# sparisi/pvr_habitat

Measured on AMD Instinct MI355X. Metric: frames/sec embedded (ResNet50, 256x256), higher is better.
Workload: dtype f16; 1 GPU; configs[1]: ResNet50 (MoCo-v2 layout) frozen, 256x256 uint8 frames resident in HBM, batch 256/GPU, random-init synthetic weights, f16 storage / MFMA inputs with fp32 accumulation (the product default, inside the 1e-3 parity bound; configs[1] names bf16); global_batch=256, frame=256, chunk=256, batches_in_flight=2, parallelism=frame shards, no collective (dp1)

## Files before the change

include/pvr_hip.h:

```cpp
#ifndef PVR_HIP_H
#define PVR_HIP_H

#include <stddef.h>
#include <stdint.h>

#ifdef __cplusplus
extern "C" {
#endif

typedef int pvr_status;
#define PVR_OK 0
#define PVR_ERR_INVALID 1
#define PVR_ERR_MISSING_WEIGHT 2
#define PVR_ERR_HIP 3
#define PVR_ERR_STATE 4

#define PVR_BF16 0
#define PVR_F16 1
#define PVR_F32 2

#define PVR_ARCH_RESNET50 0
#define PVR_ARCH_RESNET50_L4 1
#define PVR_ARCH_RESNET50_L3 2
#define PVR_ARCH_CLIP_VIT_B32 3
// ... 72 lines not shown
                                        const void *w1f_dev, const float *b1f_dev, int32_t n, int32_t dtype, uint64_t *stamps_dev, void *hip_stream);
int64_t pvr_debug_bneck_frame_launches(void);
pvr_status pvr_debug_set_frame64(int32_t mode);
int64_t pvr_debug_bneck_frame64_launches(void);
pvr_status pvr_debug_bneck_frame64_stamps(const void *w1f_dev, const float *b1f_dev, const void *w2_dev, const float *b2_dev, const void *w3_dev, const float *b3_dev,
                                          const void *x_dev, void *y_dev, int32_t n, int32_t dtype, uint64_t *stamps_dev, void *hip_stream);
pvr_status pvr_op_conv_wfrag(const void *in_dev, const void *wgt_packed_dev, const float *bias_dev, const void *residual_dev, void *out_dev, int32_t n,
                             int32_t h, int32_t w, int32_t cin, int32_t cout, int32_t kh, int32_t kw, int32_t stride, int32_t pad, int32_t relu,
                             int32_t out_f32, int32_t dtype, void *hip_stream);
pvr_status pvr_op_conv2d_dual(const void *in_dev, const void *in2_dev, const void *wgt_dev, const float *bias_dev, void *out_dev, int32_t n, int32_t h,
                              int32_t w, int32_t cin, int32_t cout, int32_t kh, int32_t kw, int32_t stride, int32_t pad, int32_t h2, int32_t w2,
                              int32_t cin2, int32_t stride2, int32_t relu, int32_t dtype, void *hip_stream);
pvr_status pvr_op_conv_wfrag_pool(const void *in_dev, const void *wgt_packed_dev, const float *bias_dev, const void *residual_dev, float *pool_out_dev,
                                  int64_t pool_stride, int32_t n, int32_t cin, int32_t cout, int32_t dtype, void *hip_stream);
int64_t pvr_debug_conv_wfrag_launches(void);
pvr_status pvr_op_split16_pack_weights(const float *w_dev, void *out_dev, int32_t rows, int32_t k, void *hip_stream);
pvr_status pvr_op_conv2d_split16(const float *in_dev, const void *wgt_split_dev, const float *bias_dev, const float *residual_dev, float *out_dev, int32_t n,
                                 int32_t h, int32_t w, int32_t cin, int32_t cout, int32_t k, int32_t stride, int32_t pad, int32_t relu, void *hip_stream);
pvr_status pvr_op_conv2d_f32(const float *in_dev, const float *wgt_dev, const float *bias_dev, const float *residual_dev, float *out_dev, int32_t n,
                             int32_t h, int32_t w, int32_t cin, int32_t cout, int32_t k, int32_t stride, int32_t pad, int32_t relu, void *hip_stream);
int64_t pvr_debug_conv_split16_launches(void);
int64_t pvr_debug_chain_wave128_launches(void);
pvr_status pvr_debug_set_conv_algo(int32_t algo);
pvr_status pvr_file_sizes(const char *const *paths, int32_t n, int64_t *sizes, int32_t threads);
pvr_status pvr_read_files(const char *const *paths, int32_t n, uint8_t *dst, const int64_t *offsets, int32_t threads);
pvr_status pvr_stage_copy(void *dst, const void *src, int64_t rows, int64_t row_bytes, int64_t src_row_stride, int64_t run_bytes,
                          int64_t run_stride, int32_t threads);
int64_t pvr_png_scratch_bytes(int32_t n, int32_t h, int32_t w);
pvr_status pvr_png_decode(const uint8_t *files_dev, const int64_t *offsets_dev, int32_t n, int32_t h, int32_t w, uint8_t *out_dev,
                          uint8_t *scratch_dev, int64_t scratch_bytes, int32_t *status_dev, void *hip_stream);
// ... 15 lines not shown
```

pvr_habitat_amd/_lib.py:

```python
import ctypes as C
import os

_HERE = os.path.dirname(os.path.abspath(__file__))
LIB_PATH = os.environ.get('PVR_LIB') or os.path.join(_HERE, 'lib', 'libpvr_hip.so')

PVR_BF16, PVR_F16, PVR_F32 = 0, 1, 2
ARCH_RESNET50, ARCH_RESNET50_L4, ARCH_RESNET50_L3 = 0, 1, 2


class EncoderDesc(C.Structure):
    _fields_ = [('arch', C.c_int32), ('dtype', C.c_int32), ('max_batch', C.c_int32), ('chunk', C.c_int32),
                ('resize', C.c_int32), ('crop', C.c_int32), ('mean', C.c_float * 3), ('std_', C.c_float * 3)]


_lib = None

_SIGS = {
    'pvr_version': (C.c_char_p, []),
    'pvr_has_experiments': (C.c_int32, []),
    'pvr_debug_stem_u8_geometry_ok': (C.c_int32, [C.c_void_p, C.c_int32, C.c_int32, C.c_int32, C.c_int32]),
    'pvr_encoder_set_host_backend': (C.c_int, [C.c_void_p, C.c_int32]),
    'pvr_stage_copy': (C.c_int, [C.c_void_p, C.c_void_p, C.c_int64, C.c_int64, C.c_int64, C.c_int64, C.c_int64, C.c_int32]),
    'pvr_last_error': (C.c_size_t, [C.c_char_p, C.c_size_t]),
    'pvr_encoder_create': (C.c_int, [C.POINTER(EncoderDesc), C.POINTER(C.c_void_p)]),
# ... 21 lines not shown
    'pvr_encoder_profile_span': (C.c_int, [C.c_void_p, C.c_void_p, C.c_int32, C.c_int32, C.c_int32, C.c_void_p, C.c_int64, C.c_void_p, C.c_int32, C.c_int32,
                                           C.POINTER(C.c_float)]),
    'pvr_op_preprocess': (C.c_int, [C.c_void_p, C.c_int32, C.c_int32, C.c_int32, C.c_int32, C.c_int32, C.c_void_p, C.c_int32, C.c_void_p]),
    'pvr_op_stem': (C.c_int, [C.c_void_p, C.c_void_p, C.c_void_p, C.c_void_p, C.c_int32, C.c_int32, C.c_void_p]),
    'pvr_op_maxpool': (C.c_int, [C.c_void_p, C.c_void_p, C.c_int32, C.c_int32, C.c_int32, C.c_int32, C.c_int32, C.c_void_p]),
    'pvr_op_conv2d': (C.c_int, [C.c_void_p, C.c_void_p, C.c_void_p, C.c_void_p, C.c_void_p] + [C.c_int32] * 12 + [C.c_void_p]),
    'pvr_op_avgpool': (C.c_int, [C.c_void_p, C.c_void_p, C.c_int64, C.c_int32, C.c_int32, C.c_int32, C.c_int32, C.c_int32, C.c_void_p]),
    'pvr_debug_convert': (C.c_int, [C.c_void_p, C.c_void_p, C.c_int64, C.c_int32]),
    'pvr_op_bneck_frame': (C.c_int, [C.c_void_p] * 13 + [C.c_int32] * 3 + [C.c_void_p]),
    'pvr_debug_bneck_frame_launches': (C.c_int64, []),
    'pvr_debug_set_frame64': (C.c_int, [C.c_int32]),
    'pvr_debug_bneck_frame64_launches': (C.c_int64, []),
    'pvr_debug_bneck_frame64_stamps': (C.c_int, [C.c_void_p] * 8 + [C.c_int32] * 2 + [C.c_void_p] * 2),
    'pvr_op_conv_wfrag': (C.c_int, [C.c_void_p] * 5 + [C.c_int32] * 12 + [C.c_void_p]),
    'pvr_debug_conv_wfrag_launches': (C.c_int64, []),
    'pvr_op_conv_wfrag_pool': (C.c_int, [C.c_void_p] * 5 + [C.c_int64] + [C.c_int32] * 4 + [C.c_void_p]),
    'pvr_op_conv2d_dual': (C.c_int, [C.c_void_p] * 5 + [C.c_int32] * 15 + [C.c_void_p]),
    'pvr_op_pack_frag_weights': (C.c_int, [C.c_void_p, C.c_void_p, C.c_int32, C.c_int32, C.c_void_p]),
    'pvr_debug_bneck_frame_stamps': (C.c_int, [C.c_void_p] * 12 + [C.c_int32] * 2 + [C.c_void_p] * 2),
    'pvr_encoder_check_range': (C.c_int, [C.c_void_p, C.c_void_p, C.c_int32, C.c_int32, C.c_int32, C.c_void_p, C.c_int64, C.c_void_p, C.POINTER(C.c_int32)]),
    'pvr_encoder_debug_set_switch': (C.c_int, [C.c_void_p, C.c_char_p, C.c_int32]),
    'pvr_encoder_launch_kernel': (C.c_int32, [C.c_void_p, C.c_int32, C.c_int32, C.c_char_p, C.c_int32]),
    'pvr_op_split16_pack_weights': (C.c_int, [C.c_void_p, C.c_void_p, C.c_int32, C.c_int32, C.c_void_p]),
    'pvr_op_conv2d_split16': (C.c_int, [C.c_void_p] * 5 + [C.c_int32] * 9 + [C.c_void_p]),
    'pvr_op_conv2d_f32': (C.c_int, [C.c_void_p] * 5 + [C.c_int32] * 9 + [C.c_void_p]),
    'pvr_debug_conv_split16_launches': (C.c_int64, []),
    'pvr_debug_chain_wave128_launches': (C.c_int64, []),
    'pvr_op_nonfinite_flag': (C.c_int, [C.c_void_p, C.c_int64, C.c_int64, C.c_int64, C.c_void_p, C.c_void_p]),
}

# ... 38 lines not shown
```

pvr_habitat_amd/csrc/api.hip:

```cpp
#include <stdarg.h>
#include "encoder_internal.h"
#include "sample_rng.h"
#include <dlfcn.h>

namespace pvr {

static thread_local std::string g_err;

void set_error(const char *fmt, ...) {
    char buf[1024];
    va_list ap;
    va_start(ap, fmt);
    vsnprintf(buf, sizeof buf, fmt, ap);
    va_end(ap);
    g_err = buf;
}
const std::string &last_error() { return g_err; }

namespace {
typedef int (*roctx_push_fn)(const char *);
typedef int (*roctx_pop_fn)();
struct Roctx {
    roctx_push_fn push = nullptr;
    roctx_pop_fn pop = nullptr;
// ... 7 lines not shown
                if (push && pop) return;
                push = nullptr; pop = nullptr;
            }
        }
    }
};
const Roctx &roctx() { static Roctx r; return r; }
}
void trace_push(const char *name) { if (roctx().push) roctx().push(name); }
void trace_pop() { if (roctx().pop) roctx().pop(); }

long long conv_expand_launches();
long long bneck_frame_launches();
long long pp_persistent_launches();
long long conv_wfrag_launches();
long long conv_split16_launches();
long long chain_wave128_launches();
pvr_status launch_split16_pack(const float *w, void *out, int rows, int K, hipStream_t stream);
pvr_status launch_conv_split16(const float *in, const void *wsp, const float *bias, const float *res, float *out, int n, int h, int w, int cin,
                               int cout, int k, int stride, int pad, int relu, hipStream_t stream, float *out2 = nullptr, int n1 = 0, void *out16 = nullptr,
                               int terms = 3);

static void *g_zero = nullptr;
static pvr_status zero_page(void **out) {
    if (!g_zero) {
        PVR_HIP_TRY(hipMalloc(&g_zero, 256));
        PVR_HIP_TRY(hipMemset(g_zero, 0, 256));
        PVR_HIP_TRY(hipDeviceSynchronize());
    }
    *out = g_zero;
// ... 47 lines not shown
}
pvr_status pvr_op_conv2d_dual(const void *in, const void *in2, const void *wgt, const float *bias, void *out, int32_t n, int32_t h, int32_t w, int32_t cin,
                              int32_t cout, int32_t kh, int32_t kw, int32_t stride, int32_t pad, int32_t h2, int32_t w2, int32_t cin2, int32_t stride2,
                              int32_t relu, int32_t dtype, void *stream) {
    PVR_REQUIRE(in && in2 && wgt && bias && out && n > 0, "pvr_op_conv2d_dual: null argument");
    PVR_REQUIRE(dtype == PVR_BF16 || dtype == PVR_F16, "pvr_op_conv2d_dual: 16-bit storage types only");
    return launch_conv_pp256(op_switches(), in, wgt, bias, nullptr, out, n, h, w, cin, cout, kh, kw, stride, pad, relu, 0, 0, dtype, 224, (hipStream_t)stream, in2, h2, w2,
                             cin2, stride2);
}
pvr_status pvr_op_conv_wfrag_pool(const void *in, const void *wgt_packed, const float *bias, const void *residual, float *pool_out, int64_t pool_stride,
                                  int32_t n, int32_t cin, int32_t cout, int32_t dtype, void *stream) {
    PVR_REQUIRE(n > 0 && pool_out, "pvr_op_conv_wfrag_pool: empty input");
    return launch_conv_wfrag(op_switches(), in, wgt_packed, bias, residual, nullptr, n, 7, 7, cin, cout, 1, 1, 1, 0, 1, 1, dtype, (hipStream_t)stream, pool_out, pool_stride);
}
int64_t pvr_debug_conv_wfrag_launches(void) { return (int64_t)conv_wfrag_launches(); }
pvr_status pvr_op_split16_pack_weights(const float *w, void *out, int32_t rows, int32_t k, void *stream) {
    return launch_split16_pack(w, out, rows, k, (hipStream_t)stream);
}
pvr_status pvr_op_conv2d_split16(const float *in, const void *wgt_split, const float *bias, const float *residual, float *out, int32_t n, int32_t h,
                                 int32_t w, int32_t cin, int32_t cout, int32_t k, int32_t stride, int32_t pad, int32_t relu, void *stream) {
    PVR_REQUIRE(n > 0 && h > 0 && w > 0, "pvr_op_conv2d_split16: empty input");
    return launch_conv_split16(in, wgt_split, bias, residual, out, n, h, w, cin, cout, k, stride, pad, relu, (hipStream_t)stream);
}
pvr_status pvr_op_conv2d_f32(const float *in, const float *wgt, const float *bias, const float *residual, float *out, int32_t n, int32_t h, int32_t w,
                             int32_t cin, int32_t cout, int32_t k, int32_t stride, int32_t pad, int32_t relu, void *stream) {
    PVR_REQUIRE(in && wgt && bias && out && n > 0, "pvr_op_conv2d_f32: null argument");
    return launch_conv_f32(in, wgt, bias, residual, out, n, h, w, cin, cout, k, stride, pad, relu, (hipStream_t)stream);
}
int64_t pvr_debug_conv_split16_launches(void) { return (int64_t)conv_split16_launches(); }
int64_t pvr_debug_chain_wave128_launches(void) { return (int64_t)chain_wave128_launches(); }
// ... 98 lines not shown
```

pvr_habitat_amd/csrc/conv_wfrag.hip:

```cpp
#include "encoder_internal.h"

namespace pvr {

struct WFP {
    const u16 *in, *w, *res;
    const float *bias;
    void *out;
    int M, H, W, Cin, Cout, Ho, Wo, KH, KW, stride, pad, act;
    int MT, NCT;
    int nch, cpt;
    int KC;
    int ct_major;
    unsigned in_bytes, w_bytes, out_bytes, res_bytes;
    float *pool_out;
    long long pool_stride;
    int frames;
};

#define WF_LDS_PTR(off_) ((__attribute__((address_space(3))) void *)(smem + (off_)))

template <bool F16, int RES, bool OUT32, int KO = 0, bool POOL = false>
__global__ __launch_bounds__(512, 1) void conv_wfrag_kernel(WFP p) {
    typedef typename HT<F16>::V8 V8;
    constexpr int BMV = POOL ? 98 : 112;
    constexpr int BM = 112, NT = 7, XB = 16384;
    constexpr int OOB = 0x7ffffff0;
    extern __shared__ __attribute__((aligned(16))) char smem[];

    const int tid = threadIdx.x, lane = tid & 63;
    const int wave = __builtin_amdgcn_readfirstlane(tid >> 6);
    const int fr = lane & 15, fq = lane >> 4, sw = (fr >> 1) & 7;
    const int t = xcd_remap(blockIdx.x, gridDim.x);
    int mt, ct;
    if (p.ct_major) { ct = t / p.MT; mt = t - ct * p.MT; }
    else { mt = t / p.NCT; ct = t - mt * p.NCT; }
    const int m0 = mt * BMV, co0 = ct * 256;

    const auto rs_in = __builtin_amdgcn_make_buffer_rsrc(const_cast<u16 *>(p.in), 0, p.in_bytes, 0x00020000);
    const auto rs_w = __builtin_amdgcn_make_buffer_rsrc(const_cast<u16 *>(p.w), 0, p.w_bytes, 0x00020000);

    int a_off[2], a_m[2];
#pragma unroll
    for (int i = 0; i < 2; ++i) {
        const int g = wave + 8 * i, r = g * 8 + (lane >> 3);
        const int lch = (lane & 7) ^ ((r >> 1) & 7);
        const int m = m0 + r;
        const bool ok = g < BM / 8 && r < BMV && m < p.M;
        const int mm = ok ? m : 0;
        const int wo = mm % p.Wo, tq = mm / p.Wo, ho = tq % p.Ho, n = tq / p.Ho;
        const int hi0 = ho * p.stride - p.pad, wi0 = wo * p.stride - p.pad;
        a_off[i] = (((n * p.H + hi0) * p.W + wi0) * p.Cin + lch * 8) * 2;
// ... 71 lines not shown
    {                                                                                                          \
        asm volatile("s_waitcnt vmcnt(6)" ::: "memory");                                                        \
        if constexpr (!(KO & 4)) __builtin_amdgcn_s_barrier();                                                  \
        __builtin_amdgcn_sched_barrier(0);                                                                      \
        WF_LOAD_W1(WF_, 0, 0) WF_STEP(0, B_, BN_, W_)                                                           \
        WF_LOAD_W1(WF_, 0, 1) WF_STEP(1, B_, BN_, W_)                                                           \
        WF_LOAD_W1(WF_, 1, 0) WF_STEP(2, B_, BN_, W_)                                                           \
        WF_LOAD_W1(WF_, 1, 1) WF_STEP(3, B_, BN_, W_)                                                           \
        if (w_c + 1 < p.nch) ++w_c;                                                                             \
        WF_STAGE1(BF_, 0) WF_STEP(4, B_, BN_, W_)                                                               \
        WF_STAGE1(BF_, 1) WF_STEP(5, B_, BN_, W_)                                                               \
        WF_STAGE_NEXT(1);                                                                                       \
        WF_STEP(6, B_, BN_, W_)                                                                                 \
    }

    const int c = co0 + 32 * wave + 8 * fq;
    u32x4 rr[NT];
    if constexpr (RES == 1) {
        const auto rs_r = __builtin_amdgcn_make_buffer_rsrc(const_cast<u16 *>(p.res), 0, p.res_bytes, 0x00020000);
#pragma unroll
        for (int j = 0; j < NT; ++j) {
            const int m = m0 + 16 * j + fr;
            rr[j] = __builtin_bit_cast(u32x4, __builtin_amdgcn_raw_buffer_load_b128(rs_r, (m < p.M && 16 * j + fr < BMV) ? (m * p.Cout + c) * 2 : OOB, 0, 0));
        }
        asm volatile("" ::: "memory");
    }
    WF_STAGE_NEXT(0); WF_LOAD_W_(w0, true); WF_STAGE(0);
    WF_STAGE_NEXT(1); WF_LOAD_W_(w1, true); WF_STAGE(1);
    WF_STAGE_NEXT(1); WF_LOAD_W_(w2, true); WF_STAGE(2);
    if constexpr ((KO & 2) != 0) WF_LOAD_W_(w3, true);
    WF_STAGE_NEXT(1);
    asm volatile("s_waitcnt vmcnt(12)" ::: "memory");
    __builtin_amdgcn_s_barrier();
    __builtin_amdgcn_sched_barrier(0);
    WF_XREAD(0, 0); WF_XREAD(1, 0); WF_XREAD(2, 0);
#pragma unroll 1
    for (int c = 0;; c += 4) {
        WF_ITER(0, 1, 3, w0, w3);
        if (c + 1 >= p.nch) break;
        WF_ITER(1, 2, 0, w1, w0);
        if (c + 2 >= p.nch) break;
        WF_ITER(2, 3, 1, w2, w1);
        if (c + 3 >= p.nch) break;
        WF_ITER(3, 0, 2, w3, w2);
        if (c + 4 >= p.nch) break;
    }
    asm volatile("s_waitcnt lgkmcnt(0)" ::: "memory");
    __builtin_amdgcn_sched_barrier(0);

    const f32x4 bl = *reinterpret_cast<const f32x4 *>(p.bias + c), bh = *reinterpret_cast<const f32x4 *>(p.bias + c + 4);
    const auto rs_o = __builtin_amdgcn_make_buffer_rsrc(p.out, 0, p.out_bytes, 0x00020000);
    float ps[2][8];
#pragma unroll
    for (int f = 0; f < 2; ++f)
#pragma unroll
        for (int e = 0; e < 8; ++e) ps[f][e] = 0.f;
#pragma unroll
    for (int j = 0; j < NT; ++j) {
        const int m = m0 + 16 * j + fr;
        const f32x4 lo = acc[0][j], hi = acc[1][j];
        float v[8] = {lo[0] + bl[0], lo[1] + bl[1], lo[2] + bl[2], lo[3] + bl[3], hi[0] + bh[0], hi[1] + bh[1], hi[2] + bh[2], hi[3] + bh[3]};
        if constexpr (RES == 1) {
#pragma unroll
            for (int e = 0; e < 4; ++e) {
                v[2 * e] += from_h<F16>((u16)(rr[j][e] & 0xffffu));
                v[2 * e + 1] += from_h<F16>((u16)(rr[j][e] >> 16));
            }
        }
        if (p.act) {
#pragma unroll
            for (int e = 0; e < 8; ++e) v[e] = fmaxf(v[e], 0.f);
        }
        if constexpr (POOL) {
            const int pp = 16 * j + fr;
#pragma unroll
            for (int e = 0; e < 8; ++e) {
                ps[0][e] += pp < 49 ? v[e] : 0.f;
                ps[1][e] += (pp >= 49 && pp < 98) ? v[e] : 0.f;
            }
        } else if constexpr (OUT32) {
            const int o = m < p.M ? (m * p.Cout + c) * 4 : OOB;
            __builtin_amdgcn_raw_buffer_store_b128(__builtin_bit_cast(u32x4, f32x4{v[0], v[1], v[2], v[3]}), rs_o, o, 0, 0);
            __builtin_amdgcn_raw_buffer_store_b128(__builtin_bit_cast(u32x4, f32x4{v[4], v[5], v[6], v[7]}), rs_o, o, 16, 0);
        } else {
            u32x4 o;
#pragma unroll
            for (int e = 0; e < 4; ++e) o[e] = (unsigned)to_h<F16>(v[2 * e]) | ((unsigned)to_h<F16>(v[2 * e + 1]) << 16);
            __builtin_amdgcn_raw_buffer_store_b128(o, rs_o, m < p.M ? (m * p.Cout + c) * 2 : OOB, 0, 0);
        }
    }
    if constexpr (POOL) {
#pragma unroll
        for (int f = 0; f < 2; ++f) {
            float tot[8];
#pragma unroll
            for (int e = 0; e < 8; ++e) {
                float t = ps[f][e];
                if (f == 1) t = __builtin_bit_cast(float, __builtin_amdgcn_update_dpp(0, __builtin_bit_cast(int, t), 0x12f, 0xf, 0xf, false));
                t += __builtin_bit_cast(float, __builtin_amdgcn_update_dpp(0, __builtin_bit_cast(int, t), 0x111, 0xf, 0xf, true));
                t += __builtin_bit_cast(float, __builtin_amdgcn_update_dpp(0, __builtin_bit_cast(int, t), 0x112, 0xf, 0xf, true));
                t += __builtin_bit_cast(float, __builtin_amdgcn_update_dpp(0, __builtin_bit_cast(int, t), 0x114, 0xf, 0xf, true));
                t += __builtin_bit_cast(float, __builtin_amdgcn_update_dpp(0, __builtin_bit_cast(int, t), 0x118, 0xf, 0xf, true));
                tot[e] = t / 49.f;
            }
            const int frame = 2 * mt + f;
            if (fr == 15 && frame < p.frames) {
                float *o = p.pool_out + (long long)frame * p.pool_stride + c;
                *reinterpret_cast<f32x4 *>(o) = f32x4{tot[0], tot[1], tot[2], tot[3]};
                *reinterpret_cast<f32x4 *>(o + 4) = f32x4{tot[4], tot[5], tot[6], tot[7]};
            }
        }
    }
#undef WF_ITER
#undef WF_STEP
#undef WF_XREAD
#undef WF_LOAD_W1
#undef WF_LOAD_W_
#undef WF_LOAD_W
#undef WF_STAGE
#undef WF_STAGE1
#undef WF_STAGE_NEXT
}

static long long g_conv_wfrag_launches = 0;
long long conv_wfrag_launches() { return g_conv_wfrag_launches; }

bool conv_wfrag_supported(int64_t M, int64_t in_bytes, int cin, int cout, int kh, int kw, int pad, int act, int out_f32) {
    const int64_t K = (int64_t)kh * kw * cin;
    return cin % 64 == 0 && cout % 256 == 0 && kh <= 3 && kh == kw && (pad == kh / 2 || pad == 0) && (act == 0 || act == 1) && !(out_f32 & 2) && M >= 1 &&
           M * cout * ((out_f32 & 1) ? 4 : 2) < 0x7ffffff0ll && in_bytes < 0x7ffffff0ll && (int64_t)cout * K * 2 < 0x7ffffff0ll;
}

bool conv_wfrag_preferred(const PlanSwitches &sw, int64_t M, int cin, int cout, int kh, int kw) {
    const int on = sw.conv_wfrag;
    const int64_t K = (int64_t)kh * kw * cin, nct = cout / 256, t256 = ((M + 255) / 256) * nct, t112 = ((M + 111) / 112) * nct;
    if (on == 2) return K >= 512;
    return on && K >= 1024 && t256 < 160 && t112 >= 192;
}

pvr_status launch_conv_wfrag(const PlanSwitches &sw, const void *in, const void *wp, const float *bias, const void *res, void *out, int n, int h, int w, int cin, int cout,
                             int kh, int kw, int stride, int pad, int act, int out_f32, int dtype, hipStream_t stream, float *pool_out, int64_t pool_stride) {
    PVR_REQUIRE(in && wp && bias && (out || pool_out), "conv_wfrag: null argument");
    PVR_REQUIRE(dtype == PVR_BF16 || dtype == PVR_F16, "conv_wfrag: 16-bit storage types only");
    const int ho = (h + 2 * pad - kh) / stride + 1, wo = (w + 2 * pad - kw) / stride + 1;
    const int64_t M = (int64_t)n * ho * wo;
    PVR_REQUIRE(conv_wfrag_supported(M, (int64_t)n * h * w * cin * 2, cin, cout, kh, kw, pad, act, out_f32), "conv_wfrag: unsupported shape");
    WFP p;
    p.in = (const u16 *)in; p.w = (const u16 *)wp; p.res = (const u16 *)res; p.bias = bias; p.out = out;
    p.M = (int)M; p.H = h; p.W = w; p.Cin = cin; p.Cout = cout; p.Ho = ho; p.Wo = wo; p.KH = kh; p.KW = kw; p.stride = stride; p.pad = pad; p.act = act;
    p.MT = pool_out ? (n + 1) / 2 : (int)((M + 111) / 112); p.NCT = cout / 256;
    p.pool_out = pool_out; p.pool_stride = pool_stride; p.frames = n;
    PVR_REQUIRE(!pool_out || (ho == 7 && wo == 7 && res && act == 1 && pool_stride >= cout && ((size_t)pool_out & 15) == 0 && pool_stride % 4 == 0),
                "conv_wfrag: the pooled form is the 7 x 7 conv3 + identity + ReLU of the trunk's last block");
    p.cpt = cin / 64; p.nch = kh * kw * p.cpt; p.KC = kh * kw * cin / 8;
    const int64_t wbytes = (int64_t)cout * kh * kw * cin * 2;
    p.ct_major = wbytes > (5 << 19) ? 1 : 0;
    p.in_bytes = (unsigned)((int64_t)n * h * w * cin * 2); p.w_bytes = (unsigned)wbytes;
    p.out_bytes = (unsigned)(M * cout * ((out_f32 & 1) ? 4 : 2)); p.res_bytes = res ? (unsigned)(M * cout * 2) : 0;
    constexpr int lds = 4 * 16384;
    const dim3 grid((unsigned)(p.MT * p.NCT)), block(512);
    ++g_conv_wfrag_launches;
    const bool f16 = dtype == PVR_F16, o32 = out_f32 & 1;
#define WF_GO(F_, R_, O_) hipLaunchKernelGGL((conv_wfrag_kernel<F_, R_, O_>), grid, block, lds, stream, p)
#ifdef PVR_EXPERIMENTS
    if (sw.wfrag_ko && dtype == PVR_F16 && !res && !(out_f32 & 1)) {
#define WF_KO(k_) case k_: hipLaunchKernelGGL((conv_wfrag_kernel<true, 0, false, k_>), grid, block, lds, stream, p); break;
        switch (sw.wfrag_ko) { WF_KO(1) WF_KO(2) WF_KO(3) WF_KO(4) WF_KO(7) WF_KO(8) WF_KO(9) WF_KO(10) WF_KO(11) WF_KO(15) default: break; }
#undef WF_KO
        PVR_LAUNCH_CHECK();
        return PVR_OK;
    }
#endif
    if (pool_out) {
        if (f16) hipLaunchKernelGGL((conv_wfrag_kernel<true, 1, false, 0, true>), grid, block, lds, stream, p);
        else hipLaunchKernelGGL((conv_wfrag_kernel<false, 1, false, 0, true>), grid, block, lds, stream, p);
        PVR_LAUNCH_CHECK();
        return PVR_OK;
    }
    if (f16) {
        if (res) { if (o32) WF_GO(true, 1, true); else WF_GO(true, 1, false); }
        else { if (o32) WF_GO(true, 0, true); else WF_GO(true, 0, false); }
    } else {
        if (res) { if (o32) WF_GO(false, 1, true); else WF_GO(false, 1, false); }
        else { if (o32) WF_GO(false, 0, true); else WF_GO(false, 0, false); }
    }
#undef WF_GO
    PVR_LAUNCH_CHECK();
// ... 5 lines not shown
```

pvr_habitat_amd/csrc/encoder.hip:

```cpp
#include "encoder_internal.h"

namespace pvr {

pvr_status launch_split16_pack(const float *w, void *out, int rows, int K, hipStream_t stream);
pvr_status launch_conv_split16(const float *in, const void *wsp, const float *bias, const float *res, float *out, int n, int h, int w, int cin,
                               int cout, int k, int stride, int pad, int relu, hipStream_t stream, float *out2 = nullptr, int n1 = 0, void *out16 = nullptr,
                               int terms = 3);

void read_switches(PlanSwitches &sw) {
    auto get = [](const char *name, int def) { const char *v = getenv(name); return v ? atoi(v) : def; };
    sw.pool_fuse = get("PVR_POOL_FUSE", 1);
    sw.stem_u8 = get("PVR_STEM_U8", 1);
    sw.stem_lds = get("PVR_STEM_LDS", 1);
    sw.stem_regpool = get("PVR_STEM_REGPOOL", 1);
    sw.frame_front1 = get("PVR_FRAME_FRONT1", 1);
    sw.frame_next1 = get("PVR_FRAME_NEXT1", 0);
    sw.frame_bneck = get("PVR_FRAME_BNECK", 1);
    sw.frame64 = get("PVR_FRAME64", 0);
    sw.bneck_stagger = get("PVR_FRAME_STAGGER", 0);
    sw.dual_ds = get("PVR_DUAL_DS", 1);
    sw.chain_ds = get("PVR_CHAIN_DS", 1);
    sw.chain_blocked = get("PVR_CHAIN_BLOCKED", 1);
    sw.chain_halo = get("PVR_CHAIN_HALO", 1);
    sw.chain_ds_occ = get("PVR_CHAIN_DS_OCC", 3);
// ... 8 lines not shown
    sw.smallk_div = get("PVR_SMALLK_DIV", 4);
    if (sw.smallk_div < 1) sw.smallk_div = 1;
    sw.frame_min_n = get("PVR_FRAME_MIN_N", 128);
    sw.frame_run = get("PVR_FRAME_RUN", 0);
    sw.frame_stagger = get("PVR_FRAME_RUN_STAGGER", 0);
    sw.split16 = get("PVR_SPLIT16", 1);
    sw.stem_conv1 = get("PVR_STEM_CONV1", 1);
    sw.resid32 = get("PVR_RESID32", 1);
    sw.tail_f32 = get("PVR_TAIL_F32", 1);
    sw.fuse = get("PVR_FUSE", 1);
    sw.conv_algo = get("PVR_CONV_ALGO", -1);
    sw.conv_halo = get("PVR_CONV_HALO", 1);
    sw.conv_expand = get("PVR_CONV_EXPAND", 1);
    sw.conv_wfrag = get("PVR_CONV_WFRAG", 1);
    sw.wfrag_ko = get("PVR_WFRAG_KO", 0);
    sw.igemm_nk4 = get("PVR_IGEMM_NK4", 1);
    sw.igemm_bm64 = get("PVR_IGEMM_BM64", 0);
    sw.pp_bm224 = get("PVR_PP_BM224", 1);
    sw.pp_persist = get("PVR_PP_PERSIST", 384);
}

PlanSwitches &op_switches() {
    static PlanSwitches sw = [] { PlanSwitches v; read_switches(v); return v; }();
    return sw;
}

template <bool F32>
__global__ __launch_bounds__(256) void range_flag_kernel(const void *x, size_t n8, int dtype, int *flags, int idx) {
    bool bad = false;
    for (size_t i = (size_t)blockIdx.x * 256 + threadIdx.x; i < n8; i += (size_t)gridDim.x * 256) {
// ... 811 lines not shown
    if (!enc->vit && !enc->rnd && !enc->host) resolve_kinds(enc);
    return PVR_OK;
}

pvr_status pvr_encoder_debug_set_switch(pvr_encoder *enc, const char *name, int32_t value) {
    PVR_REQUIRE(enc && name, "pvr_encoder_debug_set_switch: null argument");
    const std::string nm = name;
    if (nm == "pool_fuse") enc->sw.pool_fuse = value;
    else if (nm == "stem_u8") enc->sw.stem_u8 = value;
    else if (nm == "frame_min_n") enc->sw.frame_min_n = value;
    else if (nm == "frame_run") enc->sw.frame_run = value;
    else if (nm == "frame_stagger") enc->sw.frame_stagger = value;
    else if (nm == "conv_algo") enc->sw.conv_algo = value;
    else if (nm == "frame64") enc->sw.frame64 = value;
    else if (nm == "stem_regpool") enc->sw.stem_regpool = value;
    else {
        set_error("pvr_encoder_debug_set_switch: '%s' is not a live switch (pool_fuse, stem_u8, frame_min_n, frame_run, frame_stagger, conv_algo, frame64, "
                  "stem_regpool); plan switches are read from the environment at create", name);
        return PVR_ERR_INVALID;
    }
    if (!enc->vit && !enc->rnd && !enc->host) resolve_kinds(enc);
    return PVR_OK;
}

pvr_status pvr_encoder_check_range(pvr_encoder *enc, const uint8_t *frames, int32_t n, int32_t h, int32_t w, float *out, int64_t out_stride, void *hip_stream,
                                   int32_t *first_bad) {
    PVR_REQUIRE(enc && frames && out && first_bad, "pvr_encoder_check_range: null argument");
    PVR_NO_HOST(enc, "pvr_encoder_check_range");
    PVR_REQUIRE(enc->finalized && !enc->vit && !enc->rnd && enc->desc.arch != PVR_ARCH_CLIP_RN50 && enc->desc.dtype != PVR_F32,
                "pvr_encoder_check_range: built for the 16-bit plans of the torchvision ResNet family");
    PVR_REQUIRE(n > 0 && n <= enc->desc.chunk, "pvr_encoder_check_range: n=%d must fit one chunk (%d)", n, enc->desc.chunk);
    hipStream_t st = (hipStream_t)hip_stream;
    const size_t nl = enc->sched_plain.size();
// ... 104 lines not shown
```

pvr_habitat_amd/csrc/encoder_internal.h:

```cpp
#pragma once
#include <map>
#include <string>
#include <vector>
#include <cmath>
#include "common.h"
#include "chain_params.h"

namespace pvr {

struct PlanSwitches {
    int pool_fuse = 1;
    int stem_u8 = 1;
    int stem_lds = 1;
    int stem_regpool = 1;
    int frame_front1 = 1;
    int frame_next1 = 0;
    int frame_bneck = 1;
    int frame64 = 0;
    int bneck_stagger = 0;
    int dual_ds = 1;
    int chain_ds = 1;
    int chain_blocked = 1;
    int chain_halo = 1;
    int chain_ds_occ = 3;
// ... 7 lines not shown
    int splitk = 1;
    int smallk_div = 4;
    int frame_run = 0;
    int frame_stagger = 0;
    int frame_min_n = 128;
    int stem_conv1 = 1;
    int split16 = 1;
    int resid32 = 1;
    int tail_f32 = 1;
    int fuse = 1;
    int conv_algo = -1;
    int conv_halo = 1;
    int conv_expand = 1;
    int conv_wfrag = 1;
    int wfrag_ko = 0;
    int igemm_nk4 = 1;
    int igemm_bm64 = 0;
    int pp_bm224 = 1;
    int pp_persist = 384;
};
void read_switches(PlanSwitches &sw);
PlanSwitches &op_switches();

pvr_status launch_preprocess(const uint8_t *, int, int, int, int, int, void *, int, hipStream_t, int crop_pos = 0);
pvr_status launch_stem(const void *, const void *, const float *, void *, int, int, int, hipStream_t);
pvr_status launch_maxpool(const void *, void *, int, int, int, int, int, hipStream_t);
pvr_status launch_stem_pool(const PlanSwitches &sw, const void *, const void *, const float *, void *, int, int, int, hipStream_t, const void *c1_w = nullptr,
                            const float *c1_b = nullptr, void *c1_t1 = nullptr, int c1_blk = 0);
bool stem_pool_u8_ok(const void *, int, int, int, int);
pvr_status launch_stem_pool_u8(const PlanSwitches &sw, const uint8_t *, int, int, int, int, int, const void *, const float *, void *, int, hipStream_t,
// ... 27 lines not shown
struct BFBlk {
    const unsigned short *w1f, *w2, *w3, *res;
    const float *b1f, *b2, *b3;
    unsigned short *y;
};
pvr_status launch_bneck_frame_run(const BFBlk *blocks, int nblk, int n, int dtype, hipStream_t stream, int stagger);
pvr_status launch_bneck_frame64(const void *w1p, const float *b1, const void *w2p, const float *b2, const void *w3p, const float *b3, const void *x, void *y, int n,
                                int dtype, hipStream_t stream, unsigned long long *stamps);
long long bneck_frame64_launches();

bool conv_wfrag_supported(int64_t M, int64_t in_bytes, int cin, int cout, int kh, int kw, int pad, int act, int out_f32);
bool conv_wfrag_preferred(const PlanSwitches &sw, int64_t M, int cin, int cout, int kh, int kw);
pvr_status launch_conv_wfrag(const PlanSwitches &sw, const void *in, const void *wp, const float *bias, const void *res, void *out, int n, int h, int w, int cin, int cout,
                             int kh, int kw, int stride, int pad, int act, int out_f32, int dtype, hipStream_t stream, float *pool_out = nullptr,
                             int64_t pool_stride = 0);

struct HostTensor {
    std::vector<int64_t> shape;
    std::vector<float> data;
};

constexpr int PVR_MAX_LANES = 4;
enum BufId { B_NONE = -1, B_X0 = 0, B_X1, B_T1, B_T2, B_DS, B_F32, B_Y0, B_Y1, B_COUNT, B_STEM = B_COUNT };

struct ConvOp {
    std::string conv, bn;
    int in_buf, out_buf, res_buf;
    int h, w, cin, cin_real, cout, cout_real, k, stride, pad, relu, out_f32;
    int kind = 0;
    bool f32op = false;
// ... 152 lines not shown
```

Baseline: 99470 frames/s.

## Add LDS-resident 3x3 layer4 conv form and grouped-cout pooled conv3 form

Adds two new forms of the wfrag conv kernel, both enabled by default. FORM 1 handles the 7x7, 512-channel 3x3 conv: it loads two whole frames (98 rows) into LDS once and builds each of the 9 taps from shifted row addresses, with a sentinel zero row for padding, instead of staging im2col tiles per K chunk. FORM 2 handles the pooled final conv3: each workgroup keeps its input tile in LDS and loops over G output-channel groups, which reuses the staged activations and reduces the number of workgroups. The trade-offs are large dynamic LDS use with one workgroup per CU, fewer tiles to spread across the GPU, and new hand-scheduled waitcnt code that must be correct.

```diff
diff --git a/include/pvr_hip.h b/include/pvr_hip.h
--- a/include/pvr_hip.h
+++ b/include/pvr_hip.h
@@ -110,6 +110,9 @@
 pvr_status pvr_op_conv_wfrag_pool(const void *in_dev, const void *wgt_packed_dev, const float *bias_dev, const void *residual_dev, float *pool_out_dev,
                                   int64_t pool_stride, int32_t n, int32_t cin, int32_t cout, int32_t dtype, void *hip_stream);
 int64_t pvr_debug_conv_wfrag_launches(void);
+pvr_status pvr_debug_set_wfrag_resident(int32_t mode);
+int64_t pvr_debug_conv_wfrag_resident_launches(void);
+int32_t pvr_debug_wfrag_resident_row(int32_t row, int32_t tap);
 pvr_status pvr_op_split16_pack_weights(const float *w_dev, void *out_dev, int32_t rows, int32_t k, void *hip_stream);
 pvr_status pvr_op_conv2d_split16(const float *in_dev, const void *wgt_split_dev, const float *bias_dev, const float *residual_dev, float *out_dev, int32_t n,
                                  int32_t h, int32_t w, int32_t cin, int32_t cout, int32_t k, int32_t stride, int32_t pad, int32_t relu, void *hip_stream);
diff --git a/pvr_habitat_amd/_lib.py b/pvr_habitat_amd/_lib.py
--- a/pvr_habitat_amd/_lib.py
+++ b/pvr_habitat_amd/_lib.py
@@ -59,6 +59,9 @@
     'pvr_debug_bneck_frame64_stamps': (C.c_int, [C.c_void_p] * 8 + [C.c_int32] * 2 + [C.c_void_p] * 2),
     'pvr_op_conv_wfrag': (C.c_int, [C.c_void_p] * 5 + [C.c_int32] * 12 + [C.c_void_p]),
     'pvr_debug_conv_wfrag_launches': (C.c_int64, []),
+    'pvr_debug_set_wfrag_resident': (C.c_int, [C.c_int32]),
+    'pvr_debug_conv_wfrag_resident_launches': (C.c_int64, []),
+    'pvr_debug_wfrag_resident_row': (C.c_int32, [C.c_int32, C.c_int32]),
     'pvr_op_conv_wfrag_pool': (C.c_int, [C.c_void_p] * 5 + [C.c_int64] + [C.c_int32] * 4 + [C.c_void_p]),
     'pvr_op_conv2d_dual': (C.c_int, [C.c_void_p] * 5 + [C.c_int32] * 15 + [C.c_void_p]),
     'pvr_op_pack_frag_weights': (C.c_int, [C.c_void_p, C.c_void_p, C.c_int32, C.c_int32, C.c_void_p]),
diff --git a/pvr_habitat_amd/csrc/api.hip b/pvr_habitat_amd/csrc/api.hip
--- a/pvr_habitat_amd/csrc/api.hip
+++ b/pvr_habitat_amd/csrc/api.hip
@@ -45,6 +45,7 @@
 long long bneck_frame_launches();
 long long pp_persistent_launches();
 long long conv_wfrag_launches();
+long long conv_wfrag_resident_launches();
 long long conv_split16_launches();
 long long chain_wave128_launches();
 pvr_status launch_split16_pack(const float *w, void *out, int rows, int K, hipStream_t stream);
@@ -122,6 +123,14 @@
     return launch_conv_wfrag(op_switches(), in, wgt_packed, bias, residual, nullptr, n, 7, 7, cin, cout, 1, 1, 1, 0, 1, 1, dtype, (hipStream_t)stream, pool_out, pool_stride);
 }
 int64_t pvr_debug_conv_wfrag_launches(void) { return (int64_t)conv_wfrag_launches(); }
+pvr_status pvr_debug_set_wfrag_resident(int32_t mode) {
+    PVR_REQUIRE(mode >= -1 && mode <= 3, "pvr_debug_set_wfrag_resident: -1 (environment: PVR_WFRAG_RESIDENT, default on), 0, 1, or 2 / 3 (one form only)");
+    if (mode < 0) { PlanSwitches env; read_switches(env); mode = env.wfrag_resident; }
+    op_switches().wfrag_resident = mode;
+    return PVR_OK;
+}
+int64_t pvr_debug_conv_wfrag_resident_launches(void) { return (int64_t)conv_wfrag_resident_launches(); }
+int32_t pvr_debug_wfrag_resident_row(int32_t row, int32_t tap) { return wfrag_resident_row(row, tap); }
 pvr_status pvr_op_split16_pack_weights(const float *w, void *out, int32_t rows, int32_t k, void *stream) {
     return launch_split16_pack(w, out, rows, k, (hipStream_t)stream);
 }
diff --git a/pvr_habitat_amd/csrc/conv_wfrag.hip b/pvr_habitat_amd/csrc/conv_wfrag.hip
--- a/pvr_habitat_amd/csrc/conv_wfrag.hip
+++ b/pvr_habitat_amd/csrc/conv_wfrag.hip
@@ -8,6 +8,7 @@
     void *out;
     int M, H, W, Cin, Cout, Ho, Wo, KH, KW, stride, pad, act;
     int MT, NCT;
+    int G;
     int nch, cpt;
     int KC;
     int ct_major;
@@ -19,10 +20,10 @@
 
 #define WF_LDS_PTR(off_) ((__attribute__((address_space(3))) void *)(smem + (off_)))
 
-template <bool F16, int RES, bool OUT32, int KO = 0, bool POOL = false>
+template <bool F16, int RES, bool OUT32, int KO = 0, bool POOL = false, int FORM = 0>
 __global__ __launch_bounds__(512, 1) void conv_wfrag_kernel(WFP p) {
     typedef typename HT<F16>::V8 V8;
-    constexpr int BMV = POOL ? 98 : 112;
+    constexpr int BMV = (POOL || FORM == 1) ? 98 : 112;
     constexpr int BM = 112, NT = 7, XB = 16384;
     constexpr int OOB = 0x7ffffff0;
     extern __shared__ __attribute__((aligned(16))) char smem[];
@@ -34,7 +35,7 @@
     int mt, ct;
     if (p.ct_major) { ct = t / p.MT; mt = t - ct * p.MT; }
     else { mt = t / p.NCT; ct = t - mt * p.NCT; }
-    const int m0 = mt * BMV, co0 = ct * 256;
+    const int m0 = mt * BMV, co0 = ct * 256 * (FORM == 2 ? p.G : 1);
 
     const auto rs_in = __builtin_amdgcn_make_buffer_rsrc(const_cast<u16 *>(p.in), 0, p.in_bytes, 0x00020000);
     const auto rs_w = __builtin_amdgcn_make_buffer_rsrc(const_cast<u16 *>(p.w), 0, p.w_bytes, 0x00020000);
@@ -136,41 +137,19 @@
         WF_STEP(6, B_, BN_, W_)                                                                                 \
     }
 
-    const int c = co0 + 32 * wave + 8 * fq;
+    int c = co0 + 32 * wave + 8 * fq;
     u32x4 rr[NT];
-    if constexpr (RES == 1) {
-        const auto rs_r = __builtin_amdgcn_make_buffer_rsrc(const_cast<u16 *>(p.res), 0, p.res_bytes, 0x00020000);
-#pragma unroll
-        for (int j = 0; j < NT; ++j) {
-            const int m = m0 + 16 * j + fr;
-            rr[j] = __builtin_bit_cast(u32x4, __builtin_amdgcn_raw_buffer_load_b128(rs_r, (m < p.M && 16 * j + fr < BMV) ? (m * p.Cout + c) * 2 : OOB, 0, 0));
-        }
-        asm volatile("" ::: "memory");
-    }
-    WF_STAGE_NEXT(0); WF_LOAD_W_(w0, true); WF_STAGE(0);
-    WF_STAGE_NEXT(1); WF_LOAD_W_(w1, true); WF_STAGE(1);
-    WF_STAGE_NEXT(1); WF_LOAD_W_(w2, true); WF_STAGE(2);
-    if constexpr ((KO & 2) != 0) WF_LOAD_W_(w3, true);
-    WF_STAGE_NEXT(1);
-    asm volatile("s_waitcnt vmcnt(12)" ::: "memory");
-    __builtin_amdgcn_s_barrier();
-    __builtin_amdgcn_sched_barrier(0);
-    WF_XREAD(0, 0); WF_XREAD(1, 0); WF_XREAD(2, 0);
-#pragma unroll 1
-    for (int c = 0;; c += 4) {
-        WF_ITER(0, 1, 3, w0, w3);
-        if (c + 1 >= p.nch) break;
-        WF_ITER(1, 2, 0, w1, w0);
-        if (c + 2 >= p.nch) break;
-        WF_ITER(2, 3, 1, w2, w1);
-        if (c + 3 >= p.nch) break;
-        WF_ITER(3, 0, 2, w3, w2);
-        if (c + 4 >= p.nch) break;
-    }
-    asm volatile("s_waitcnt lgkmcnt(0)" ::: "memory");
-    __builtin_amdgcn_sched_barrier(0);
-
-    const f32x4 bl = *reinterpret_cast<const f32x4 *>(p.bias + c), bh = *reinterpret_cast<const f32x4 *>(p.bias + c + 4);
+#define WF_LOAD_RES()                                                                                           \
+    {                                                                                                          \
+        const auto rs_r = __builtin_amdgcn_make_buffer_rsrc(const_cast<u16 *>(p.res), 0, p.res_bytes, 0x00020000);   \
+        _Pragma("unroll") for (int j = 0; j < NT; ++j) {                                                        \
+            const int m = m0 + 16 * j + fr;                                                                     \
+            rr[j] = __builtin_bit_cast(u32x4, __builtin_amdgcn_raw_buffer_load_b128(rs_r, (m < p.M && 16 * j + fr < BMV) ? (m * p.Cout + c) * 2 : OOB, 0, 0));   \
+        }                                                                                                       \
+        asm volatile("" ::: "memory");                                                                          \
+    }
+    if constexpr (RES == 1 && FORM != 2) WF_LOAD_RES()
+    auto epilogue = [&](const int c, const f32x4 bl, const f32x4 bh) __attribute__((always_inline)) {
     const auto rs_o = __builtin_amdgcn_make_buffer_rsrc(p.out, 0, p.out_bytes, 0x00020000);
     float ps[2][8];
 #pragma unroll
@@ -201,14 +180,14 @@
                 ps[1][e] += (pp >= 49 && pp < 98) ? v[e] : 0.f;
             }
         } else if constexpr (OUT32) {
-            const int o = m < p.M ? (m * p.Cout + c) * 4 : OOB;
+            const int o = (m < p.M && (BMV == BM || 16 * j + fr < BMV)) ? (m * p.Cout + c) * 4 : OOB;
             __builtin_amdgcn_raw_buffer_store_b128(__builtin_bit_cast(u32x4, f32x4{v[0], v[1], v[2], v[3]}), rs_o, o, 0, 0);
             __builtin_amdgcn_raw_buffer_store_b128(__builtin_bit_cast(u32x4, f32x4{v[4], v[5], v[6], v[7]}), rs_o, o, 16, 0);
         } else {
             u32x4 o;
 #pragma unroll
             for (int e = 0; e < 4; ++e) o[e] = (unsigned)to_h<F16>(v[2 * e]) | ((unsigned)to_h<F16>(v[2 * e + 1]) << 16);
-            __builtin_amdgcn_raw_buffer_store_b128(o, rs_o, m < p.M ? (m * p.Cout + c) * 2 : OOB, 0, 0);
+            __builtin_amdgcn_raw_buffer_store_b128(o, rs_o, (m < p.M && (BMV == BM || 16 * j + fr < BMV)) ? (m * p.Cout + c) * 2 : OOB, 0, 0);
         }
     }
     if constexpr (POOL) {
@@ -233,19 +212,190 @@
             }
         }
     }
+    };
+    if constexpr (FORM == 1) {
+        constexpr int RROW = 1152;
+#pragma unroll
+        for (int i = 0; i < 13; ++i) {
+            const int r = wave + 8 * i;
+            const int lch = (lane & 7) ^ ((r >> 1) & 7);
+            const int m = m0 + r;
+            const int src = (r < 98 && m < p.M) ? (m * 512 + (lane >> 3) * 64 + lch * 8) * 2 : OOB;
+            __builtin_amdgcn_raw_ptr_buffer_load_lds(rs_in, WF_LDS_PTR(r * RROW), 16, src, 0, 0, 0);
+            asm volatile("" ::: "memory");
+        }
+        int vm[NT];
+#pragma unroll
+        for (int j = 0; j < NT; ++j) {
+            vm[j] = 0;
+#pragma unroll
+            for (int t9 = 0; t9 < 9; ++t9) vm[j] |= (int)(wfrag_resident_row(16 * j + fr, t9) != WFRAG_ZERO_ROW) << t9;
+        }
+        int ra[NT], rb[NT];
+#define WR_ADDR(tap_)                                                                                           \
+    {                                                                                                          \
+        const int tp_ = (tap_) < 9 ? (tap_) : 8, ky_ = tp_ / 3, d_ = (ky_ - 1) * 7 + (tp_ - 3 * ky_ - 1);       \
+        _Pragma("unroll") for (int j = 0; j < NT; ++j) {                                                        \
+            const int lr_ = ((vm[j] >> tp_) & 1) ? 16 * j + fr + d_ : WFRAG_ZERO_ROW;                           \
+            ra[j] = lr_ * RROW + ((fq ^ ((lr_ >> 1) & 7)) << 4);                                                \
+            rb[j] = ra[j] ^ 64;                                                                                 \
+        }                                                                                                       \
+    }
+#define WR_XREAD(j_, S_)                                                                                        \
+    {                                                                                                          \
+        asm volatile("ds_read_b128 %0, %1 offset:%2" : "=v"(xs[j_][0]) : "v"(ra[j_]), "n"((S_) * 128));         \
+        asm volatile("ds_read_b128 %0, %1 offset:%2" : "=v"(xs[j_][1]) : "v"(rb[j_]), "n"((S_) * 128));         \
+    }
+#define WR_STEP(q_, S_, SN_, W_)                                                                                \
+    {                                                                                                          \
+        if ((q_) + RD < NT) WR_XREAD((q_) + RD, S_) else WR_XREAD((q_) + RD - NT, SN_);                         \
+        asm volatile("s_waitcnt lgkmcnt(6)" : "+v"(xs[q_][0]), "+v"(xs[q_][1]));                                \
+        __builtin_amdgcn_sched_barrier(0);                                                                      \
+        acc[0][q_] = mfma16<F16>(W_[0][0], xs[q_][0], acc[0][q_]);                                              \
+        acc[1][q_] = mfma16<F16>(W_[1][0], xs[q_][0], acc[1][q_]);                                              \
+        acc[0][q_] = mfma16<F16>(W_[0][1], xs[q_][1], acc[0][q_]);                                              \
+        acc[1][q_] = mfma16<F16>(W_[1][1], xs[q_][1], acc[1][q_]);                                              \
+    }
+#define WR_ITER(S_, W_, WF_)                                                                                    \
+    {                                                                                                          \
+        asm volatile("s_waitcnt vmcnt(8)" ::: "memory");                                                        \
+        __builtin_amdgcn_sched_barrier(0);                                                                      \
+        WF_LOAD_W1(WF_, 0, 0) WR_STEP(0, S_, ((S_) + 1) & 7, W_)                                                \
+        WF_LOAD_W1(WF_, 0, 1) WR_STEP(1, S_, ((S_) + 1) & 7, W_)                                                \
+        WF_LOAD_W1(WF_, 1, 0) WR_STEP(2, S_, ((S_) + 1) & 7, W_)                                                \
+        WF_LOAD_W1(WF_, 1, 1) WR_STEP(3, S_, ((S_) + 1) & 7, W_)                                                \
+        if (w_c + 1 < p.nch) ++w_c;                                                                             \
+        if constexpr ((S_) == 7) WR_ADDR(tap + 1)                                                               \
+        WR_STEP(4, S_, ((S_) + 1) & 7, W_)                                                                      \
+        WR_STEP(5, S_, ((S_) + 1) & 7, W_)                                                                      \
+        WR_STEP(6, S_, ((S_) + 1) & 7, W_)                                                                      \
+    }
+        WF_LOAD_W_(w0, true); WF_LOAD_W_(w1, true); WF_LOAD_W_(w2, true);
+        WR_ADDR(0)
+        asm volatile("s_waitcnt vmcnt(12)" ::: "memory");
+        __builtin_amdgcn_s_barrier();
+        __builtin_amdgcn_sched_barrier(0);
+        WR_XREAD(0, 0); WR_XREAD(1, 0); WR_XREAD(2, 0);
+#pragma unroll 1
+        for (int tap = 0; tap < 9; ++tap) {
+            WR_ITER(0, w0, w3); WR_ITER(1, w1, w0); WR_ITER(2, w2, w1); WR_ITER(3, w3, w2);
+            WR_ITER(4, w0, w3); WR_ITER(5, w1, w0); WR_ITER(6, w2, w1); WR_ITER(7, w3, w2);
+        }
+#undef WR_ITER
+#undef WR_STEP
+#undef WR_XREAD
+#undef WR_ADDR
+    } else if constexpr (FORM == 2) {
+        WF_STAGE_NEXT(0); WF_STAGE(0);
+        WF_STAGE_NEXT(1); WF_STAGE(1); WF_STAGE_NEXT(1); WF_STAGE(2); WF_STAGE_NEXT(1); WF_STAGE(3);
+        WF_STAGE_NEXT(1); WF_STAGE(4); WF_STAGE_NEXT(1); WF_STAGE(5); WF_STAGE_NEXT(1); WF_STAGE(6); WF_STAGE_NEXT(1); WF_STAGE(7);
+        const int KC = p.KC, wg_last = 8 * p.G - 1;
+        int wg = 0;
+#define WP_LOAD_W1(dst_, i_, ks_)                                                                               \
+    {                                                                                                          \
+        dst_[i_][ks_] = __builtin_bit_cast(V8, __builtin_amdgcn_raw_buffer_load_b128(rs_w, wlane, ((rt0 + 16 * (wg >> 3) + (i_)) * KC + 4 * (2 * (wg & 7) + (ks_))) * 256, 0));   \
+        asm volatile("" ::: "memory");                                                                          \
+    }
+#define WP_LOAD_W(dst_) { WP_LOAD_W1(dst_, 0, 0) WP_LOAD_W1(dst_, 0, 1) WP_LOAD_W1(dst_, 1, 0) WP_LOAD_W1(dst_, 1, 1) if (wg < wg_last) ++wg; }
+        const int xcH = xc + 4 * XB, xcH64 = xc64 + 4 * XB;
+#define WP_XREAD(j_, B_)                                                                                        \
+    {                                                                                                          \
+        asm volatile("ds_read_b128 %0, %1 offset:%2" : "=v"(xs[j_][0]) : "v"((B_) < 4 ? xc : xcH), "n"(((B_) & 3) * XB + (j_) * 2048));     \
+        asm volatile("ds_read_b128 %0, %1 offset:%2" : "=v"(xs[j_][1]) : "v"((B_) < 4 ? xc64 : xcH64), "n"(((B_) & 3) * XB + (j_) * 2048)); \
+    }
+#define WP_STEP(q_, B_, W_)                                                                                     \
+    {                                                                                                          \
+        if ((q_) + RD < NT) WP_XREAD((q_) + RD, B_) else WP_XREAD((q_) + RD - NT, ((B_) + 1) & 7);              \
+        asm volatile("s_waitcnt lgkmcnt(6)" : "+v"(xs[q_][0]), "+v"(xs[q_][1]));                                \
+        __builtin_amdgcn_sched_barrier(0);                                                                      \
+        acc[0][q_] = mfma16<F16>(W_[0][0], xs[q_][0], acc[0][q_]);                                              \
+        acc[1][q_] = mfma16<F16>(W_[1][0], xs[q_][0], acc[1][q_]);                                              \
+        acc[0][q_] = mfma16<F16>(W_[0][1], xs[q_][1], acc[0][q_]);                                              \
+        acc[1][q_] = mfma16<F16>(W_[1][1], xs[q_][1], acc[1][q_]);                                              \
+    }
+#define WP_ITER(B_, W_, WF_)                                                                                    \
+    {                                                                                                          \
+        __builtin_amdgcn_sched_barrier(0);                                                                      \
+        WP_LOAD_W1(WF_, 0, 0) WP_STEP(0, B_, W_)                                                                \
+        WP_LOAD_W1(WF_, 0, 1) WP_STEP(1, B_, W_)                                                                \
+        WP_LOAD_W1(WF_, 1, 0) WP_STEP(2, B_, W_)                                                                \
+        WP_LOAD_W1(WF_, 1, 1) WP_STEP(3, B_, W_)                                                                \
+        if (wg < wg_last) ++wg;                                                                                 \
+        WP_STEP(4, B_, W_) WP_STEP(5, B_, W_) WP_STEP(6, B_, W_)                                                \
+    }
+        WP_LOAD_W(w0) WP_LOAD_W(w1) WP_LOAD_W(w2)
+        asm volatile("s_waitcnt vmcnt(12)" ::: "memory");
+        __builtin_amdgcn_s_barrier();
+        __builtin_amdgcn_sched_barrier(0);
+        WP_XREAD(0, 0); WP_XREAD(1, 0); WP_XREAD(2, 0);
+#pragma unroll 1
+        for (int g = 0; g < p.G; ++g) {
+            if constexpr (RES == 1) WF_LOAD_RES()
+            const f32x4 bl = *reinterpret_cast<const f32x4 *>(p.bias + c), bh = *reinterpret_cast<const f32x4 *>(p.bias + c + 4);
+            asm volatile("" ::: "memory");
+            WP_ITER(0, w0, w3); WP_ITER(1, w1, w0); WP_ITER(2, w2, w1); WP_ITER(3, w3, w2);
+            WP_ITER(4, w0, w3); WP_ITER(5, w1, w0); WP_ITER(6, w2, w1); WP_ITER(7, w3, w2);
+            epilogue(c, bl, bh);
+#pragma unroll
+            for (int i = 0; i < 2; ++i)
+#pragma unroll
+                for (int j = 0; j < NT; ++j) acc[i][j] = f32x4{0.f, 0.f, 0.f, 0.f};
+            c += 256;
+        }
+#undef WP_ITER
+#undef WP_STEP
+#undef WP_XREAD
+#undef WP_LOAD_W
+#undef WP_LOAD_W1
+    } else {
+        WF_STAGE_NEXT(0); WF_LOAD_W_(w0, true); WF_STAGE(0);
+        WF_STAGE_NEXT(1); WF_LOAD_W_(w1, true); WF_STAGE(1);
+        WF_STAGE_NEXT(1); WF_LOAD_W_(w2, true); WF_STAGE(2);
+        if constexpr ((KO & 2) != 0) WF_LOAD_W_(w3, true);
+        WF_STAGE_NEXT(1);
+        asm volatile("s_waitcnt vmcnt(12)" ::: "memory");
+        __builtin_amdgcn_s_barrier();
+        __builtin_amdgcn_sched_barrier(0);
+        WF_XREAD(0, 0); WF_XREAD(1, 0); WF_XREAD(2, 0);
+    #pragma unroll 1
+        for (int c = 0;; c += 4) {
+            WF_ITER(0, 1, 3, w0, w3);
+            if (c + 1 >= p.nch) break;
+            WF_ITER(1, 2, 0, w1, w0);
+            if (c + 2 >= p.nch) break;
+            WF_ITER(2, 3, 1, w2, w1);
+            if (c + 3 >= p.nch) break;
+            WF_ITER(3, 0, 2, w3, w2);
+            if (c + 4 >= p.nch) break;
+        }
+    }
+    asm volatile("s_waitcnt lgkmcnt(0)" ::: "memory");
+    __builtin_amdgcn_sched_barrier(0);
+
+    if constexpr (FORM != 2) {
+        const f32x4 bl = *reinterpret_cast<const f32x4 *>(p.bias + c), bh = *reinterpret_cast<const f32x4 *>(p.bias + c + 4);
+        epilogue(c, bl, bh);
+    }
 #undef WF_ITER
 #undef WF_STEP
 #undef WF_XREAD
 #undef WF_LOAD_W1
 #undef WF_LOAD_W_
 #undef WF_LOAD_W
+#undef WF_LOAD_RES
 #undef WF_STAGE
 #undef WF_STAGE1
 #undef WF_STAGE_NEXT
 }
 
-static long long g_conv_wfrag_launches = 0;
+static long long g_conv_wfrag_launches = 0, g_conv_wfrag_resident_launches = 0;
 long long conv_wfrag_launches() { return g_conv_wfrag_launches; }
+long long conv_wfrag_resident_launches() { return g_conv_wfrag_resident_launches; }
+
+static bool wfrag_resident_shape(const PlanSwitches &sw, int h, int w, int cin, int kh, int kw, int stride, int pad, const void *res, int out_f32, const float *pool_out) {
+    return (sw.wfrag_resident & 1) && !pool_out && !res && !(out_f32 & 1) && h == 7 && w == 7 && cin == 512 && kh == 3 && kw == 3 && stride == 1 && pad == 1;
+}
+constexpr int WFRAG_RESIDENT_LDS = 104 * 1152;
 
 bool conv_wfrag_supported(int64_t M, int64_t in_bytes, int cin, int cout, int kh, int kw, int pad, int act, int out_f32) {
     const int64_t K = (int64_t)kh * kw * cin;
@@ -270,7 +420,14 @@
     WFP p;
     p.in = (const u16 *)in; p.w = (const u16 *)wp; p.res = (const u16 *)res; p.bias = bias; p.out = out;
     p.M = (int)M; p.H = h; p.W = w; p.Cin = cin; p.Cout = cout; p.Ho = ho; p.Wo = wo; p.KH = kh; p.KW = kw; p.stride = stride; p.pad = pad; p.act = act;
-    p.MT = pool_out ? (n + 1) / 2 : (int)((M + 111) / 112); p.NCT = cout / 256;
+    const bool resident = wfrag_resident_shape(sw, h, w, cin, kh, kw, stride, pad, res, out_f32, pool_out);
+    const bool resident_pool = (sw.wfrag_resident == 1 || sw.wfrag_resident == 2) && pool_out && cin == 512;
+    p.MT = (pool_out || resident) ? (n + 1) / 2 : (int)((M + 111) / 112); p.NCT = cout / 256;
+    p.G = 1;
+    if (resident_pool) {
+        while (p.G * 2 <= p.NCT && p.NCT % (p.G * 2) == 0 && (int64_t)p.MT * (p.NCT / p.G) > 256) p.G *= 2;
+        p.NCT /= p.G;
+    }
     p.pool_out = pool_out; p.pool_stride = pool_stride; p.frames = n;
     PVR_REQUIRE(!pool_out || (ho == 7 && wo == 7 && res && act == 1 && pool_stride >= cout && ((size_t)pool_out & 15) == 0 && pool_stride % 4 == 0),
                 "conv_wfrag: the pooled form is the 7 x 7 conv3 + identity + ReLU of the trunk's last block");
@@ -293,6 +450,33 @@
         return PVR_OK;
     }
 #endif
+    if (resident) {
+        static bool attr_set = false;
+        if (!attr_set) {
+            PVR_HIP_TRY(hipFuncSetAttribute((const void *)conv_wfrag_kernel<true, 0, false, 0, false, 1>, hipFuncAttributeMaxDynamicSharedMemorySize, WFRAG_RESIDENT_LDS));
+            PVR_HIP_TRY(hipFuncSetAttribute((const void *)conv_wfrag_kernel<false, 0, false, 0, false, 1>, hipFuncAttributeMaxDynamicSharedMemorySize, WFRAG_RESIDENT_LDS));
+            attr_set = true;
+        }
+        ++g_conv_wfrag_resident_launches;
+        if (f16) hipLaunchKernelGGL((conv_wfrag_kernel<true, 0, false, 0, false, 1>), grid, block, WFRAG_RESIDENT_LDS, stream, p);
+        else hipLaunchKernelGGL((conv_wfrag_kernel<false, 0, false, 0, false, 1>), grid, block, WFRAG_RESIDENT_LDS, stream, p);
+        PVR_LAUNCH_CHECK();
+        return PVR_OK;
+    }
+    if (resident_pool) {
+        constexpr int lds8 = 8 * 16384;
+        static bool attr_set = false;
+        if (!attr_set) {
+            PVR_HIP_TRY(hipFuncSetAttribute((const void *)conv_wfrag_kernel<true, 1, false, 0, true, 2>, hipFuncAttributeMaxDynamicSharedMemorySize, lds8));
+            PVR_HIP_TRY(hipFuncSetAttribute((const void *)conv_wfrag_kernel<false, 1, false, 0, true, 2>, hipFuncAttributeMaxDynamicSharedMemorySize, lds8));
+            attr_set = true;
+        }
+        ++g_conv_wfrag_resident_launches;
+        if (f16) hipLaunchKernelGGL((conv_wfrag_kernel<true, 1, false, 0, true, 2>), grid, block, lds8, stream, p);
+        else hipLaunchKernelGGL((conv_wfrag_kernel<false, 1, false, 0, true, 2>), grid, block, lds8, stream, p);
+        PVR_LAUNCH_CHECK();
+        return PVR_OK;
+    }
     if (pool_out) {
         if (f16) hipLaunchKernelGGL((conv_wfrag_kernel<true, 1, false, 0, true>), grid, block, lds, stream, p);
         else hipLaunchKernelGGL((conv_wfrag_kernel<false, 1, false, 0, true>), grid, block, lds, stream, p);
diff --git a/pvr_habitat_amd/csrc/encoder.hip b/pvr_habitat_amd/csrc/encoder.hip
--- a/pvr_habitat_amd/csrc/encoder.hip
+++ b/pvr_habitat_amd/csrc/encoder.hip
@@ -46,6 +46,7 @@
     sw.conv_expand = get("PVR_CONV_EXPAND", 1);
     sw.conv_wfrag = get("PVR_CONV_WFRAG", 1);
     sw.wfrag_ko = get("PVR_WFRAG_KO", 0);
+    sw.wfrag_resident = get("PVR_WFRAG_RESIDENT", 1);
     sw.igemm_nk4 = get("PVR_IGEMM_NK4", 1);
     sw.igemm_bm64 = get("PVR_IGEMM_BM64", 0);
     sw.pp_bm224 = get("PVR_PP_BM224", 1);
@@ -887,9 +888,10 @@
     else if (nm == "conv_algo") enc->sw.conv_algo = value;
     else if (nm == "frame64") enc->sw.frame64 = value;
     else if (nm == "stem_regpool") enc->sw.stem_regpool = value;
+    else if (nm == "wfrag_resident") enc->sw.wfrag_resident = value;
     else {
         set_error("pvr_encoder_debug_set_switch: '%s' is not a live switch (pool_fuse, stem_u8, frame_min_n, frame_run, frame_stagger, conv_algo, frame64, "
-                  "stem_regpool); plan switches are read from the environment at create", name);
+                  "stem_regpool, wfrag_resident); plan switches are read from the environment at create", name);
         return PVR_ERR_INVALID;
     }
     if (!enc->vit && !enc->rnd && !enc->host) resolve_kinds(enc);
diff --git a/pvr_habitat_amd/csrc/encoder_internal.h b/pvr_habitat_amd/csrc/encoder_internal.h
--- a/pvr_habitat_amd/csrc/encoder_internal.h
+++ b/pvr_habitat_amd/csrc/encoder_internal.h
@@ -45,6 +45,7 @@
     int conv_expand = 1;
     int conv_wfrag = 1;
     int wfrag_ko = 0;
+    int wfrag_resident = 1;
     int igemm_nk4 = 1;
     int igemm_bm64 = 0;
     int pp_bm224 = 1;
@@ -102,6 +103,12 @@
 pvr_status launch_conv_wfrag(const PlanSwitches &sw, const void *in, const void *wp, const float *bias, const void *res, void *out, int n, int h, int w, int cin, int cout,
                              int kh, int kw, int stride, int pad, int act, int out_f32, int dtype, hipStream_t stream, float *pool_out = nullptr,
                              int64_t pool_stride = 0);
+constexpr int WFRAG_ZERO_ROW = 98;
+__host__ __device__ inline int wfrag_resident_row(int row, int tap) {
+    if (row < 0 || row >= 98 || tap < 0 || tap >= 9) return WFRAG_ZERO_ROW;
+    const int q = row % 49, y = q / 7 + tap / 3 - 1, x = q % 7 + tap % 3 - 1;
+    return (y >= 0 && y < 7 && x >= 0 && x < 7) ? row + (tap / 3 - 1) * 7 + tap % 3 - 1 : WFRAG_ZERO_ROW;
+}
 
 struct HostTensor {
     std::vector<int64_t> shape;
```

Measured after the change: 99950 frames/s, median of 4. About the same (+0.5%).
